# DanMcGann/loam

Measured on AMD Instinct MI355X. Metric: scan-pair registrations/sec (64x1024 Ouster), higher is better.
Workload: dtype f64; 1 GPU; batch of 1024 independent 64x1024 scan pairs per GPU (BASELINE configs[2]/[3]); step = extractFeatures x2 + registerFeatures per pair, inputs resident in HBM; pairs_per_gpu=1024, scan=64x1024, seed=20240311, input_scalar=f64, arithmetic=f64 (float input is widened on load)

## Files before the change

loam_amd/csrc/api_host.h:

```cpp
#pragma once
#include <math.h>
#include <stdio.h>
#include <stdlib.h>
#include <string.h>

#include <mutex>
#include <string>
#include <type_traits>
#include <utility>
#include <vector>

#include "loamx_internal.h"

namespace loamx {

enum WsId {
  WS_XYZ = 0, WS_CURV, WS_MASK,
  WS_SORT_SCRATCH, WS_SORT_SCRATCH_SRC, WS_NASSOC, WS_STATE, WS_PARTIALS, WS_MOM_PARTIALS, WS_MOMENTS, WS_FLAGGED_LIST, WS_FLAGGED_COUNT,
  WS_LINE_TOT, WS_EXTRACT_EVENTS, WS_BOX, WS_FINITE_FLAG, WS_COUNTERS, WS_ITERINFO, WS_STREAM_IN0, WS_STREAM_IN1, WS_STREAM_RES,
  WS_FIT_IN, WS_FIT_OUT, WS_FCOUNTS, WS_RESULTS, WS_INIT, WS_STREAM_INIT,
  WS_VOX_TABLE, WS_MAP_WORDS, WS_INFO_PARTIALS, WS_INFO,
  WS_COUNT
};
enum WsKindId {
  WSK_STAGE = 0, WSK_CNT, WSK_IDX, WSK_N, WSK_XYZ,
  WSK_GRID_DESC, WSK_CELLS, WSK_SORTED, WSK_REL, WSK_SGRID_DESC, WSK_SCELLS, WSK_SSORTED, WSK_ASSOC, WSK_NN, WSK_RNN, WSK_NEAREST,
  WSK_REST, WSK_EXACT, WSK_DUMP, WSK_SRC, WSK_TGT, WSK_MAP_TMP, WSK_MAP_OUT,
  WSK_COUNT
};

struct Buf {
  void* p = nullptr;
  size_t cap = 0;
};

struct PendingEvent {
  int kernel;
  hipEvent_t e0, e1;
  double bytes;
  bool own_e0;
};

}

struct loamx_ctx {
  int device = 0;
  hipStream_t own_stream = nullptr, stream = nullptr;
  bool max_counts_clean = false;
  hipStream_t aux_stream = nullptr;
  hipEvent_t ev_fork = nullptr, ev_mid = nullptr, ev_join = nullptr;
  hipEvent_t ev_counts = nullptr;
// ... 203 lines not shown
```

loam_amd/csrc/api_register.hip:

```cpp
#include "api_host.h"

using namespace loamx;

namespace {

int enqueue_association(loamx_ctx* ctx, const RegBatch& B, const RegConfig& C, uint32_t what = kAssocEdges | kAssocPlanes) {
  hipStream_t s = ctx->stream;
  {
    TimedScope t(ctx, LOAMX_K_ASSOC, 0.0);
    const bool side = (size_t)B.n_pairs * B.kind[kPlane].assoc_blocks >= 128;
    PendingEvent knn{};
    LaunchScope knn_ls{nullptr, nullptr, true};
    if (ctx->timing) {
      knn.kernel = LOAMX_K_KNN_PLANE, knn.bytes = 0.0, knn.own_e0 = true;
      knn.e0 = take_event(ctx), knn.e1 = take_event(ctx);
      knn_ls = LaunchScope{knn.e0, knn.e1, true};
    }
    launch_associate(B, C, s, side ? ctx->aux_stream : nullptr, side ? ctx->aux2_stream : nullptr, ctx->ev_fork, ctx->ev_mid, ctx->ev_join,
                     ctx->ev_join2, ctx->timing ? &knn_ls : nullptr, what);
    if (ctx->timing) {
      if (knn_ls.first) ctx->event_pool.push_back(knn.e0), ctx->event_pool.push_back(knn.e1);
      else ctx->pending.push_back(knn);
    }
  }
// ... 84 lines not shown
    ENSURE(ctx, b, bytes);
    if ((C.flags & kRegFlagPoison) && b.p) HIP_TRY(ctx, hipMemsetAsync(b.p, 0xFF, b.cap, ctx->stream));
    field = reinterpret_cast<std::remove_reference_t<decltype(field)>>(b.p);
    return LOAMX_OK;
  };
#define SCRATCH(buf, bytes, field)                \
  do {                                            \
    int rc_ = scratch(buf, bytes, field);         \
    if (rc_ != LOAMX_OK) return rc_;              \
  } while (0)
#define SCRATCH_K(id, bytes, field)                                                                        \
  for (int k = 0; k < 2; k++) {                                                                            \
    RegKind& K = B.kind[k];                                                                                \
    const size_t st = K.stride, km = C.kind[k].k <= 5 ? 5 : (C.kind[k].k <= 8 ? 8 : kMaxK), rec = k ? 7 : 9; \
    SCRATCH(ctx->wsk[id][k], bytes, K.field);                                                              \
  }
  SCRATCH_K(WSK_GRID_DESC, np * sizeof(GridDesc), grid.desc)
  SCRATCH_K(WSK_CELLS, (np * (size_t)(kGridCellsCap + 1) + 4) * sizeof(uint32_t), grid.cell_start)
  SCRATCH_K(WSK_SORTED, np * (st + kGridPad) * sizeof(GridPoint), grid.sorted)
  SCRATCH_K(WSK_REL, np * 3 * (st + kGridPad) * sizeof(float), grid.rel)
  SCRATCH_K(WSK_SGRID_DESC, np * sizeof(GridDesc), src_grid.desc)
  SCRATCH_K(WSK_SCELLS, np * (size_t)(kGridCellsCap + 1) * sizeof(uint32_t), src_grid.cell_start)
  SCRATCH_K(WSK_SSORTED, np * st * sizeof(GridPoint), src_grid.sorted)
  SCRATCH(ctx->ws[WS_SORT_SCRATCH], np * (es > ps ? es : ps) * sizeof(GridPoint), B.sort_scratch);
  SCRATCH(ctx->ws[WS_SORT_SCRATCH_SRC], grid_small(es > ps ? es : ps, C.flags) ? sizeof(GridPoint) : np * (es > ps ? es : ps) * sizeof(GridPoint), B.sort_scratch_src);
  SCRATCH_K(WSK_ASSOC, rec * np * st * sizeof(double), rec)
  SCRATCH_K(WSK_NN, (1 + km) * np * st * sizeof(uint32_t), nn)
  SCRATCH_K(WSK_RNN, (1 + km) * np * st * sizeof(uint32_t), rnn)
  SCRATCH_K(WSK_NEAREST, np * st * sizeof(uint32_t), nearest)
  SCRATCH_K(WSK_REST, np * st * sizeof(uint32_t), rest)
  SCRATCH_K(WSK_EXACT, np * st * sizeof(uint32_t), exact)
  SCRATCH(ctx->ws[WS_NASSOC], np * 8 * sizeof(uint32_t), B.n_assoc);
  SCRATCH(ctx->ws[WS_STATE], np * sizeof(PairState), B.state);
  SCRATCH(ctx->ws[WS_PARTIALS], np * B.blocks_per_pair * kAccSize * sizeof(double), B.partials);
  SCRATCH(ctx->ws[WS_MOM_PARTIALS], np * B.mom_blocks_per_pair * 4 * (size_t)(kMomSize + 2) * sizeof(double), B.mom_partials);
  SCRATCH(ctx->ws[WS_MOMENTS], np * (size_t)(kMomSize + 2) * sizeof(double), B.moments);
  SCRATCH(ctx->ws[WS_FLAGGED_LIST], np * (size_t)B.mom_blocks_per_pair * kSweepChunk * sizeof(uint32_t), B.flagged_list);
  SCRATCH(ctx->ws[WS_FLAGGED_COUNT], np * (size_t)B.mom_blocks_per_pair * 4 * sizeof(uint32_t), B.flagged_count);
  if (opts.want_info_partials) {
    InfoPartial* info_partials = nullptr;
    SCRATCH(ctx->ws[WS_INFO_PARTIALS], np * info_blocks_per_pair(es, ps) * sizeof(InfoPartial), info_partials);
  }
#undef SCRATCH_K
#undef SCRATCH
  {
    const bool fresh = ctx->ws[WS_COUNTERS].cap == 0;
    ENSURE(ctx, WS_COUNTERS, 128);
    untimed(ctx);
    if (fresh) HIP_TRY(ctx, hipMemsetAsync(ctx->ws[WS_COUNTERS].p, 0, 128, ctx->stream));
  }
  if (opts.want_iter_info) ENSURE(ctx, WS_ITERINFO, np * (size_t)(C.max_iterations ? C.max_iterations : 1) * sizeof(loamx_iter_info));
  B.n_active = wsp<uint32_t>(ctx, WS_COUNTERS);
  B.sweep_slots = reinterpret_cast<unsigned long long*>(wsp<unsigned char>(ctx, WS_COUNTERS) + 8);
  B.assoc_slots = B.sweep_slots + 2;
  B.grid_bytes = B.sweep_slots + 5;
  B.iter_info = opts.want_iter_info ? wsp<loamx_iter_info>(ctx, WS_ITERINFO) : nullptr;
  B.want_nearest = opts.want_nearest ? 1u : 0u;
  B.ref_moments = (C.flags & (kRegFlagNoMoments | kRegFlagNoRefMoments)) ? 0u : 1u;
  B.max_counts = wsp<uint32_t>(ctx, WS_COUNTERS) + 16;
  B.small_edge_sets = (C.flags & kRegFlagNoSmallSets) ? 0u : (!prebuilt ? 1u : (prebuilt->n[0] <= kBruteMax ? 2u : 0u));
  hipStream_t s = ctx->stream;
  untimed(ctx);
  if (!ctx->max_counts_clean) {
    const uint32_t init[6] = {0u, 0u, 0u, 0u, 0xFFFFFFFFu, 0xFFFFFFFFu};
    memcpy(&ctx->h_pinned[8], init, sizeof(init));
    HIP_TRY(ctx, hipMemcpyAsync(B.max_counts, &ctx->h_pinned[8], sizeof(init), hipMemcpyHostToDevice, s));
  }
  ctx->max_counts_clean = false;
  launch_state_init(B, C, s);
  CHECK_LAUNCH(ctx, "state_init_kernel");
  if (!ctx->ev_counts) HIP_TRY(ctx, hipEventCreateWithFlags(&ctx->ev_counts, hipEventDisableTiming));
  HIP_TRY(ctx, hipMemcpyAsync(&ctx->h_pinned[16], B.max_counts, 6 * sizeof(uint32_t), hipMemcpyDeviceToHost, s));
  HIP_TRY(ctx, hipEventRecord(ctx->ev_counts, s));

  if (prebuilt) {
    for (int k = 0; k < 2; k++) B.kind[k].grid = index_grid_set(prebuilt, k);
  }
  {
    TimedScope t(ctx, LOAMX_K_GRID, 0.0);
    const bool side = !(C.flags & kRegFlagNoGridSide) && ctx->aux_stream && !prebuilt && hipStreamWaitEvent(ctx->aux_stream, ctx->ev_counts, 0) == hipSuccess;
    if (!prebuilt) launch_grid_build_targets(B, C, s);
    launch_grid_build_sources(B, C, side ? ctx->aux_stream : s);
    if (side && hipEventRecord(ctx->ev_join, ctx->aux_stream) == hipSuccess) (void)hipStreamWaitEvent(s, ctx->ev_join, 0);
  }
  CHECK_LAUNCH(ctx, "grid_build_kernel");
// ... 435 lines not shown
```

loam_amd/csrc/info_kernels.hip:

```cpp
#include "loamx_internal.h"
#include "info_math.h"

namespace loamx {

namespace {

static_assert(sizeof(InfoPartial::s) == kInfoSums * sizeof(double), "InfoPartial holds the sums of info_math.h");
static_assert(sizeof(loamx_reg_information) == 696, "loamx.h documents the record's size");

constexpr int kInfoThreads = 256;
constexpr int kInfoItems = 16;
constexpr int kInfoChunk = kInfoThreads * kInfoItems;

__global__ void info_activate_kernel(RegBatch B) {
  const size_t pair = (size_t)blockIdx.x * blockDim.x + threadIdx.x;
  if (pair >= B.n_pairs) return;
  B.state[pair].active = 1u;
}

__global__ __launch_bounds__(kInfoThreads) void information_kernel(RegBatch B, InfoPartial* __restrict__ partials, uint32_t blocks_per_pair) {
  __shared__ double s_sum[kInfoThreads / 64][kInfoSums];
  __shared__ uint32_t s_cnt[kInfoThreads / 64][4];
  const size_t pair = blockIdx.x / blocks_per_pair;
  const uint32_t blk = blockIdx.x % blocks_per_pair;
  const uint32_t n_se_raw = B.kind[kEdge].n_src[pair * B.in_pitch], n_sp_raw = B.kind[kPlane].n_src[pair * B.in_pitch];
  const uint32_t n_se = n_se_raw < B.kind[kEdge].stride ? n_se_raw : (uint32_t)B.kind[kEdge].stride;
  const uint32_t n_sp = n_sp_raw < B.kind[kPlane].stride ? n_sp_raw : (uint32_t)B.kind[kPlane].stride;
  const uint32_t total = n_se + n_sp;
  const uint32_t base = blk * kInfoChunk;
  if (base >= total) return;
  const size_t efield = B.n_pairs * B.kind[kEdge].stride, pfield = B.n_pairs * B.kind[kPlane].stride;
  const double* __restrict__ E = B.kind[kEdge].rec + pair * B.kind[kEdge].stride;
  const double* __restrict__ Pl = B.kind[kPlane].rec + pair * B.kind[kPlane].stride;
  InfoAcc acc;
  info_acc_clear(acc);
  struct Rec {
    double f[9];
    int kind;
  };
  auto load_rec = [&](uint32_t v) {
    Rec R;
    R.kind = 0;
#pragma unroll
    for (int f = 0; f < 9; f++) R.f[f] = 0.0;
    if (v < total) {
      if (v < n_se) {
        R.kind = 1;
#pragma unroll
        for (int f = 0; f < 9; f++) R.f[f] = E[f * efield + v];
// ... 114 lines not shown
```

loam_amd/csrc/loamx_internal.h:

```cpp
#pragma once
#include <hip/hip_runtime.h>
#include <hip/hip_ext.h>
#include <stdint.h>
#include <stdio.h>

#include "../../include/loamx.h"
#include "extract_math.h"
#include "reg_math.h"

namespace loamx {

struct LaunchScope {
  hipEvent_t start, stop;
  bool first;
};
extern thread_local LaunchScope* g_launch_scope;
extern int g_debug_sync;
template <typename F, typename... Args>
inline void launch_kernel_named(const char* name, F kernel, const dim3& grid, const dim3& block, size_t shmem, hipStream_t s, Args... args) {
  LaunchScope* sc = g_launch_scope;
  if (g_debug_sync) fprintf(stderr, "[loamx] launch %s grid %u x %u block %u\n", name, grid.x, grid.y, block.x), fflush(stderr);
  if (sc) {
    hipExtLaunchKernelGGL(kernel, grid, block, (uint32_t)shmem, s, sc->first ? sc->start : nullptr, sc->stop, 0, args...);
    sc->first = false;
// ... 134 lines not shown
  uint32_t stream_planes;
  uint32_t use_moments;
  uint32_t mom_ref_on;
  double mom_ref[7];
};

constexpr int kSweepThreads = 256;
#ifndef LOAMX_SWEEP_ITEMS
#define LOAMX_SWEEP_ITEMS 16
#endif
constexpr int kSweepItems = LOAMX_SWEEP_ITEMS;
constexpr int kSweepChunk = kSweepThreads * kSweepItems;
constexpr uint32_t kEdgeCache = 320;
constexpr uint32_t kListCache = 64;
constexpr uint32_t kFlatCache = 192;

struct RegBatch {
  size_t n_pairs;
  uint32_t in_pitch;
  RegKind kind[2];
  const double* init;
  GridPoint* sort_scratch;
  GridPoint* sort_scratch_src;
  uint32_t* n_assoc;
  PairState* state;
  double* partials;
  double* mom_partials;
  double* moments;
  uint32_t mom_blocks_per_pair;
  uint32_t* flagged_list;
  uint32_t* flagged_count;
  uint32_t blocks_per_pair;
  uint32_t* n_active;
  unsigned long long* sweep_slots;
  unsigned long long* assoc_slots;
  unsigned long long* grid_bytes;
  loamx_iter_info* iter_info;
  uint32_t* max_counts;
  uint32_t want_nearest;
  uint32_t ref_moments;
  const unsigned long long* box_min;
  const unsigned long long* box_max;
  const uint32_t* box_bad;
  uint32_t src_box_offset;
  uint32_t small_edge_sets;
};

constexpr size_t kGridBigScratchBytes = 64 + ((size_t)kGridCellsCap + kGridCellsCap / 4096 + 8) * sizeof(uint32_t);
constexpr uint32_t kGridSmallCap = 20480;
constexpr uint32_t kBruteMax = 512;
constexpr uint32_t kGridMapCellsCap = 1u << 18;
inline bool grid_small(size_t stride, uint32_t reg_flags) { return stride <= kGridSmallCap && !(reg_flags & kRegFlagNoPackedGrid); }
void launch_grid_build_targets(const RegBatch& B, const RegConfig& C, hipStream_t s);
void launch_grid_build_sources(const RegBatch& B, const RegConfig& C, hipStream_t s);
constexpr uint32_t kGridBuildNone = 0u, kGridBuildPacked = 1u, kGridBuildSingle = 2u, kGridBuildBig = 3u;
struct GridBuildForm {
  uint32_t form;
  uint32_t unit_cells;
  uint32_t table_min_points;
};
GridBuildForm launch_grid_build_target(const RegBatch& B, const RegConfig& C, int kind, hipStream_t s);
void launch_grid_build_source(const RegBatch& B, const RegConfig& C, int kind, hipStream_t s);
void launch_state_init(const RegBatch& B, const RegConfig& C, hipStream_t s);
constexpr uint32_t kAssocEdges = 1u, kAssocPlanes = 2u;
void launch_associate(const RegBatch& B, const RegConfig& C, hipStream_t s, hipStream_t aux, hipStream_t aux2, hipEvent_t ev_fork,
                      hipEvent_t ev_mid, hipEvent_t ev_join, hipEvent_t ev_join2, LaunchScope* knn_scope = nullptr,
// ... 73 lines not shown
```

loam_amd/csrc/register_kernels.hip:

```cpp
#include "loamx_internal.h"

namespace loamx {

namespace {

__device__ __forceinline__ double wave_min(double v) {
#pragma unroll
  for (int off = 32; off >= 1; off >>= 1) v = fmin(v, __shfl_xor(v, off));
  return v;
}
__device__ __forceinline__ double wave_max(double v) {
#pragma unroll
  for (int off = 32; off >= 1; off >>= 1) v = fmax(v, __shfl_xor(v, off));
  return v;
}

#ifndef LOAMX_BUILD_THREADS
#define LOAMX_BUILD_THREADS 1024
#endif
constexpr int kBuildThreads = LOAMX_BUILD_THREADS;

template <bool ORDERED, bool PACKED>
__global__ __launch_bounds__(kBuildThreads) void grid_build_kernel(const double* __restrict__ pts_base,
                                                                   const uint32_t* __restrict__ n_pts, size_t stride,
// ... 549 lines not shown
  if (c <= ncell) cell_start[c] += shift[c];
  if (c < kGridPad) rel2[n_new + c] = kRelPad, rel2[stride + n_new + c] = kRelPad, rel2[2 * stride + n_new + c] = kRelPad;
  if (c == 0) desc->n_points = n_new;
}

constexpr int kRankThreads = 256;
__global__ __launch_bounds__(kRankThreads) void grid_rank_kernel(const uint32_t* __restrict__ n_pts, size_t stride,
                                                                 uint32_t in_pitch, GridSet gs,
                                                                 const GridPoint* __restrict__ scratch, const uint32_t* __restrict__ small_if) {
  const size_t pair = blockIdx.y;
  if (small_if && small_if[pair * in_pitch] <= kBruteMax) return;
  const uint32_t n_raw = n_pts[pair * in_pitch];
  const uint32_t n = n_raw < stride ? n_raw : (uint32_t)stride;
  const uint32_t p = blockIdx.x * kRankThreads + threadIdx.x;
  if (p >= n) return;
  const GridDesc g = gs.desc[pair];
  const uint32_t* __restrict__ cs = gs.cell_start + pair * (size_t)(kGridCellsCap + 1);
  const GridPoint* __restrict__ src = scratch + pair * gs.stride;
  GridPoint* __restrict__ sp = gs.sorted + pair * gs.stride;
  const GridPoint e = src[p];
  const uint32_t cell = grid_morton_of_point(g, v3(e.x, e.y, e.z));
  const uint32_t b = cs[cell], en = cs[cell + 1];
  uint32_t rank = 0;
#pragma unroll 4
  for (uint32_t j = b; j < en; j++) rank += src[j].orig < e.orig ? 1u : 0u;
  sp[b + rank] = e;
}

__global__ void state_init_kernel(RegBatch B, RegConfig C) {
  const size_t pair = (size_t)blockIdx.x * blockDim.x + threadIdx.x;
  if (pair >= B.n_pairs) return;
  PairState& S = B.state[pair];
  for (int i = 0; i < 7; i++) S.est[i] = B.init ? B.init[pair * 7 + i] : (i == 3 ? 1.0 : 0.0);
  S.active = C.max_iterations > 0 ? 1u : 0u;
  S.termination = LOAMX_MAX_ITER;
  S.iterations = 0;
  S.first_sweep = 0;
  S.stream_planes = 1;
  S.use_moments = 0;
  S.mom_ref_on = 0;
  S.lm.active = 0;
  for (int c = 0; c < 8; c++) B.n_assoc[8 * pair + c] = 0;
  if (B.max_counts) {
    const RegKind &E = B.kind[kEdge], &P = B.kind[kPlane];
    const uint32_t ne = E.n_src[pair * B.in_pitch], np = P.n_src[pair * B.in_pitch];
    atomicMax(&B.max_counts[0], ne < E.stride ? ne : (uint32_t)E.stride);
    atomicMax(&B.max_counts[1], np < P.stride ? np : (uint32_t)P.stride);
    if (E.n_tgt && P.n_tgt) {
      uint32_t te = E.n_tgt[pair * B.in_pitch], tp = P.n_tgt[pair * B.in_pitch];
      te = te < E.stride ? te : (uint32_t)E.stride, tp = tp < P.stride ? tp : (uint32_t)P.stride;
      atomicMax(&B.max_counts[2], te), atomicMax(&B.max_counts[3], tp);
      atomicMin(&B.max_counts[4], te), atomicMin(&B.max_counts[5], tp);
    }
  }
}

constexpr int kAssocThreads = 256;
#ifndef LOAMX_ASSOC_WAVES
#define LOAMX_ASSOC_WAVES 4
#endif
#ifndef LOAMX_KNN_REQUERY
#define LOAMX_KNN_REQUERY 1
#endif
#ifndef LOAMX_HANDOFF
#define LOAMX_HANDOFF 3
#endif
static_assert(!(LOAMX_HANDOFF & 2) || (LOAMX_HANDOFF & 1), "verification in the fit needs the threshold in front of the walk");
#ifndef LOAMX_ASSOC_WAVES5
#define LOAMX_ASSOC_WAVES5 (LOAMX_KNN_REQUERY ? 6 : 4)
#endif

__device__ __forceinline__ bool xcd_pair_map(uint32_t block, uint32_t blocks_per_pair, size_t n_pairs, size_t& pair,
                                             uint32_t& chunk) {
  if (n_pairs < 8) {
    pair = block / blocks_per_pair;
    chunk = block % blocks_per_pair;
  } else {
    const uint32_t xcd = block & 7u, slot = block >> 3;
    pair = (size_t)xcd + 8u * (size_t)(slot / blocks_per_pair);
    chunk = slot % blocks_per_pair;
  }
  return pair < n_pairs;
}

constexpr int kBruteTile = 256;
constexpr size_t kBruteLdsBytes = (kBruteTile + kGridPad) * sizeof(GridPoint) + ((3 * (kBruteTile + kGridPad) * sizeof(float) + 31) / 32) * 32;

template <class Coll>
__device__ __forceinline__ void brute_scan_tile(Coll& c, int k, Vec3 q, const GridPoint* s_tile, uint32_t tile, uint32_t tn) {
  for (uint32_t u = 0; u < tn; u += 4) {
    const GridPoint t0 = s_tile[u], t1 = s_tile[u + 1], t2 = s_tile[u + 2], t3 = s_tile[u + 3];
    double dx = q.x - t0.x, dy = q.y - t0.y, dz = q.z - t0.z;
    const double d0 = dx * dx + dy * dy + dz * dz;
    dx = q.x - t1.x, dy = q.y - t1.y, dz = q.z - t1.z;
    const double d1 = dx * dx + dy * dy + dz * dz;
    dx = q.x - t2.x, dy = q.y - t2.y, dz = q.z - t2.z;
    const double d2 = dx * dx + dy * dy + dz * dz;
    dx = q.x - t3.x, dy = q.y - t3.y, dz = q.z - t3.z;
    const double d3 = dx * dx + dy * dy + dz * dz;
    knn_offer4(c, k, d0, d1, d2, d3, tile + u, tn - u, t0.orig, t1.orig, t2.orig, t3.orig);
  }
}

template <bool PLANE, int KM>
__device__ __forceinline__ void knn_brute_body(const RegBatch& B, const RegConfig& C, uint32_t blocks_per_pair, uint32_t block,
                                               GridPoint* s_tile) {
  size_t pair;
  uint32_t chunk;
  if (!xcd_pair_map(block, blocks_per_pair, B.n_pairs, pair, chunk)) return;
  const PairState& S = B.state[pair];
  if (!S.active) return;
  const RegKind& K = B.kind[PLANE];
  const RegKindConfig& CK = C.kind[PLANE];
  const GridSet& gs = K.grid;
  const uint32_t n_tgt = gs.desc[pair].n_points;
  if (n_tgt > kBruteMax) return;
  const size_t stride = K.stride;
  const uint32_t n_src = K.n_src[pair * B.in_pitch];
  if (K.knn_mode == 2u && chunk == 0 && threadIdx.x == 0 && B.assoc_slots)
    atomicAdd(&B.assoc_slots[PLANE ? 1 : 0], (unsigned long long)(n_src < stride ? n_src : stride));
  if (chunk * kAssocThreads >= n_src || chunk * kAssocThreads >= stride) return;
  const uint32_t i = chunk * kAssocThreads + threadIdx.x;
  const bool has = i < n_src && i < stride;
  const GridSet& src_gs = K.src_grid;
  const GridPoint* __restrict__ sp = gs.sorted + pair * gs.stride;
  Vec3 p = v3(0, 0, 0);
  if (has) {
    const GridPoint sq = src_gs.sorted[pair * src_gs.stride + i];
    p = pose_act(S.est, v3(sq.x, sq.y, sq.z));
  }
  int k = CK.k;
  k = k < KM ? k : KM;
  const double max_dist = CK.r;
  uint32_t pos[KM];
#pragma unroll
  for (int j = 0; j < KM; j++) pos[j] = 0;
  int kept = 0;
  if (k > 0 && n_tgt > 0) {
    const double pass_max = CK.pass;
    kept = has ? -1 : 0;
    const GridDesc g = gs.desc[pair];
    if (gs.rel != nullptr && g.h > 0.0) {
// ... 74 lines not shown
      for (uint32_t tile = 0; tile < n_tgt; tile += kBruteTile) {
        const uint32_t tn = n_tgt - tile < (uint32_t)kBruteTile ? n_tgt - tile : (uint32_t)kBruteTile;
        __syncthreads();
        for (uint32_t t = threadIdx.x; t < tn + kGridPad; t += kAssocThreads) s_tile[t] = sp[tile + t];
        __syncthreads();
        if (kept < 0) brute_scan_tile(r, k, p, s_tile, tile, tn);
      }
      if (kept < 0) {
        kept = knn_finish(r, k, max_dist);
        knn_shift_positions<KM>(r.pos, k, pos);
      }
    }
  }
  if (!has) return;
  const size_t field = B.n_pairs * stride, slot = pair * stride + i;
  uint32_t* __restrict__ nn = K.nn;
  nn[slot] = (uint32_t)kept;
#pragma unroll
  for (int j = 0; j < KM; j++) nn[(1 + j) * field + slot] = pos[j];
}
template <bool PLANE, int KM>
__global__ __launch_bounds__(kAssocThreads) void associate_knn_brute_kernel(RegBatch B, RegConfig C, uint32_t blocks_per_pair) {
  __shared__ GridPoint s_tile[kBruteLdsBytes / sizeof(GridPoint)];
  knn_brute_body<PLANE, KM>(B, C, blocks_per_pair, blockIdx.x, s_tile);
}

constexpr uint32_t kQueueIndex = 0x3FFFFFFFu, kQueueWide = 0x80000000u, kQueueTied = 0x40000000u;

template <bool PLANE, int KM, int HANDOFF = 0>
__device__ __forceinline__ void knn_round1_body(const RegBatch& B, const RegConfig& C, uint32_t blocks_per_pair, uint32_t block,
                                                uint32_t* s_rows) {
  size_t pair;
  uint32_t chunk;
  if (!xcd_pair_map(block, blocks_per_pair, B.n_pairs, pair, chunk)) return;
  const uint32_t i = chunk * kAssocThreads + threadIdx.x;
  const PairState& S = B.state[pair];
  if (!S.active) return;
  const RegKind& K = B.kind[PLANE];
  const RegKindConfig& CK = C.kind[PLANE];
  const size_t stride = K.stride;
  const uint32_t n_src = K.n_src[pair * B.in_pitch];
  const GridSet &gs = K.grid, &src_gs = K.src_grid;
  if (chunk == 0 && threadIdx.x == 0 && B.assoc_slots)
    atomicAdd(&B.assoc_slots[PLANE ? 1 : 0], (unsigned long long)(n_src < stride ? n_src : stride));
  const GridDesc g = gs.desc[pair];
  if (g.n_points <= kBruteMax) return;
  if (i >= n_src || i >= stride) return;
  const GridPoint sq = src_gs.sorted[pair * src_gs.stride + i];
  const Vec3 p = pose_act(S.est, v3(sq.x, sq.y, sq.z));
  const uint32_t* __restrict__ cs = gs.cell_start + pair * (size_t)(kGridCellsCap + 1);
  const GridPoint* __restrict__ sp = gs.sorted + pair * gs.stride;
  uint32_t pos[KM];
  const float* __restrict__ rel = gs.rel + pair * 3 * gs.stride;
  const size_t field = B.n_pairs * stride;
  uint32_t word = 0;
#if LOAMX_KNN_REQUERY
  const GridPoint* __restrict__ src_pts = src_gs.sorted + pair * src_gs.stride;
  auto requery = [&](const Vec3&) -> Vec3 {
    uint32_t ii = i;
    asm volatile("" : "+v"(ii));
    const GridPoint s2 = src_pts[ii];
    return pose_act(S.est, v3(s2.x, s2.y, s2.z));
  };
  const int kept = knn_search_f32_round1<KM, false, decltype(requery), (HANDOFF & 3)>(g, cs, sp, rel, (uint32_t)gs.stride, p, CK.k,
                                             CK.r, CK.pass, pos, s_rows + threadIdx.x, kAssocThreads, requery, &word);
#else
  const int kept = knn_search_f32_round1<KM>(g, cs, sp, rel, (uint32_t)gs.stride, p, CK.k, CK.r, CK.pass, pos,
// ... 14 lines not shown
template <bool PLANE, int KM>
__global__ __launch_bounds__(kAssocThreads, KM <= 5 ? LOAMX_ASSOC_WAVES5 : LOAMX_ASSOC_WAVES) void associate_knn_kernel(RegBatch B, RegConfig C,
                                                                                         uint32_t blocks_per_pair) {
  __shared__ uint32_t s_rows[kLeanRowWords * kAssocThreads];
  knn_round1_body<PLANE, KM>(B, C, blocks_per_pair, blockIdx.x, s_rows);
}
template <int KME, int KMP>
__global__ __launch_bounds__(kAssocThreads, (KME <= 5 && KMP <= 5) ? LOAMX_ASSOC_WAVES5 : LOAMX_ASSOC_WAVES) void associate_knn_mixed_kernel(RegBatch B, RegConfig C, uint32_t blocks_edge,
                                                                                               uint32_t blocks_plane, uint32_t edge_blocks) {
  constexpr size_t kRowBytes = sizeof(uint32_t) * kLeanRowWords * kAssocThreads, kTileBytes = kBruteLdsBytes;
  __shared__ __attribute__((aligned(16))) unsigned char s_raw[kRowBytes > kTileBytes ? kRowBytes : kTileBytes];
  if (blockIdx.x < edge_blocks) knn_brute_body<false, KME>(B, C, blocks_edge, blockIdx.x, reinterpret_cast<GridPoint*>(s_raw));
  else knn_round1_body<true, KMP, LOAMX_HANDOFF>(B, C, blocks_plane, blockIdx.x - edge_blocks, reinterpret_cast<uint32_t*>(s_raw));
}

#ifndef LOAMX_REST_THREADS
#define LOAMX_REST_THREADS 64
#endif
constexpr int kRestThreads = LOAMX_REST_THREADS;
__host__ __device__ inline bool queue_leftovers_coop(const RegConfig& C, int kind) {
  return !(C.flags & kRegFlagNoCoopLeft) && C.kind[kind].r > 0.0;
}
#ifndef LOAMX_COOP_WAVES
#define LOAMX_COOP_WAVES 4
#endif
#define LOAMX_REST_WAVES(KM) ((KM) <= 8 ? 3 : 2)
constexpr int kLeftWaves = 5;
template <bool PLANE, int KM, bool ONE_STAGE>
__global__ __launch_bounds__(kRestThreads, LOAMX_REST_WAVES(KM)) void associate_knn_rest_kernel(RegBatch B, RegConfig C,
                                                                                              uint32_t blocks_per_pair) {
  constexpr bool one_stage = ONE_STAGE;
  size_t pair;
  uint32_t chunk0;
  if (!xcd_pair_map(blockIdx.x, blocks_per_pair, B.n_pairs, pair, chunk0)) return;
  const PairState& S = B.state[pair];
  if (!S.active) return;
  const uint32_t queued = B.n_assoc[8 * pair + (PLANE ? 3 : 2)];
  if (queued == 0u) return;
  __shared__ uint32_t s_rows[(ONE_STAGE ? kLeanRowWords : kLean2RowWords) * kRestThreads];
  const RegKind& K = B.kind[PLANE];
  const RegKindConfig& CK = C.kind[PLANE];
  const size_t stride = K.stride;
  const size_t field = B.n_pairs * stride;
  uint32_t* __restrict__ rnn = K.rnn;
  const uint32_t* __restrict__ rest = K.rest + pair * stride;
  uint32_t* __restrict__ left = K.exact + pair * stride;
  const GridSet &gs = K.grid, &src_gs = K.src_grid;
  const GridDesc g = gs.desc[pair];
  const uint32_t* __restrict__ cs = gs.cell_start + pair * (size_t)(kGridCellsCap + 1);
  const GridPoint* __restrict__ sp = gs.sorted + pair * gs.stride;
  const bool spread = B.n_pairs < 8 && (size_t)queued * 4 <= (size_t)blocks_per_pair * kRestThreads;
  const uint32_t t0 = spread ? chunk0 + blocks_per_pair * threadIdx.x : chunk0 * kRestThreads + threadIdx.x;
  const uint32_t dt = spread ? 0xFFFFFFFFu - t0 : blocks_per_pair * kRestThreads;
  const bool lean_set = g.n_points <= kLeanMaxPoints;
  const int kq = CK.k;
  const double max_dist = CK.r, pass_max = CK.pass;
  for (uint32_t t = t0; t < queued; t += dt) {
    const uint32_t entry = rest[t], i = entry & kQueueIndex;
    const size_t slot = pair * stride + t;
    uint32_t pos[KM];
#pragma unroll
    for (int j = 0; j < KM; j++) pos[j] = 0;
    int kept = -1;
    const bool coop = !one_stage && queue_leftovers_coop(C, PLANE);
    if (one_stage || (!(entry & kQueueTied) && ((lean_set && !(entry & kQueueWide)) || ((entry & kQueueWide) && !coop)))) {
      const GridPoint sq = src_gs.sorted[pair * src_gs.stride + i];
      const Vec3 p = pose_act(S.est, v3(sq.x, sq.y, sq.z));
      if (entry & kQueueWide)
        kept = knn_search_f32_round1<KM, true>(g, cs, sp, gs.rel + pair * 3 * gs.stride, (uint32_t)gs.stride, p, kq, max_dist, pass_max, pos,
                                                s_rows + threadIdx.x, kRestThreads);
      else if (!one_stage)
        kept = knn_lean_round2<KM>(g, cs, sp, gs.rel + pair * 3 * gs.stride, (uint32_t)gs.stride, p, kq, max_dist, pass_max, pos,
                                   s_rows + threadIdx.x, kRestThreads);
      if (one_stage && kept < 0)
        kept = knn_search_keyed<KM>(g, cs, sp, p, kq, max_dist, pass_max, pos, s_rows + threadIdx.x, kRestThreads);
    }
    rnn[slot] = (uint32_t)kept;
    if (kept < 0) left[atomicAdd(&B.n_assoc[8 * pair + (PLANE ? 5 : 4)], 1u)] = t;
#pragma unroll
    for (int j = 0; j < KM; j++) rnn[(1 + j) * field + slot] = pos[j];
  }
}

template <bool PLANE, int KM>
__global__ __launch_bounds__(kRestThreads, kLeftWaves) void associate_knn_left_kernel(RegBatch B, RegConfig C,
                                                                                              uint32_t blocks_per_pair) {
  size_t pair;
  uint32_t chunk0;
  if (!xcd_pair_map(blockIdx.x, blocks_per_pair, B.n_pairs, pair, chunk0)) return;
  const PairState& S = B.state[pair];
  if (!S.active) return;
  const uint32_t listed = B.n_assoc[8 * pair + (PLANE ? 5 : 4)];
  if (listed == 0u) return;
  __shared__ uint32_t s_rows[kLeanRowWords * kRestThreads];
  const RegKind& K = B.kind[PLANE];
  const RegKindConfig& CK = C.kind[PLANE];
  const size_t stride = K.stride;
  const size_t field = B.n_pairs * stride;
  uint32_t* __restrict__ rnn = K.rnn;
  const uint32_t* __restrict__ rest = K.rest + pair * stride;
  const uint32_t* __restrict__ left = K.exact + pair * stride;
  const GridSet &gs = K.grid, &src_gs = K.src_grid;
  const GridDesc g = gs.desc[pair];
  const uint32_t* __restrict__ cs = gs.cell_start + pair * (size_t)(kGridCellsCap + 1);
  const GridPoint* __restrict__ sp = gs.sorted + pair * gs.stride;
  const bool spread = B.n_pairs < 8 && (size_t)listed * 4 <= (size_t)blocks_per_pair * kRestThreads;
  const uint32_t t0 = spread ? chunk0 + blocks_per_pair * threadIdx.x : chunk0 * kRestThreads + threadIdx.x;
  const uint32_t dt = spread ? 0xFFFFFFFFu - t0 : blocks_per_pair * kRestThreads;
  for (uint32_t t = t0; t < listed; t += dt) {
    const uint32_t qpos = left[t], i = rest[qpos] & kQueueIndex;
    const size_t slot = pair * stride + qpos;
    const GridPoint sq = src_gs.sorted[pair * src_gs.stride + i];
    const Vec3 p = pose_act(S.est, v3(sq.x, sq.y, sq.z));
    uint32_t pos[KM];
    const int kept = knn_search_keyed<KM>(g, cs, sp, p, CK.k, CK.r, CK.pass, pos, s_rows + threadIdx.x, kRestThreads);
    rnn[slot] = (uint32_t)kept;
#pragma unroll
    for (int j = 0; j < KM; j++) rnn[(1 + j) * field + slot] = pos[j];
  }
}

constexpr int32_t kCoopMaxShell = 64;
// ... 141 lines not shown
        bound = ub < bound ? ub : bound;
      }
      done = knn_done(g, q, k, max_dist, cx, cy, cz, probe, w);
    }
  }
  if (!done) return -1;
  KnnKeys<KM> m;
  knn_init(m, k, g.n_points);
#pragma unroll
  for (int t = 0; t <= KM; t++) {
    if (t >= KM - k) {
      double head = knn_key_empty();
#pragma unroll
      for (int j = KM; j >= 0; j--)
        if (j >= KM - k) head = c.key[j] < head ? c.key[j] : head;
      const double best = wave_min_all(head);
      m.key[t] = best;
      if (head == best && best < knn_key_empty()) {
#pragma unroll
        for (int j = 0; j < KM; j++)
          if (j >= KM - k) c.key[j] = c.key[j + 1];
        c.key[KM] = knn_key_empty();
      }
    }
  }
  return knn_keys_finish(m, k, pass_max, pos);
}

static_assert(kRestThreads == 64, "associate_knn_coop_kernel is written for one wavefront per workgroup");
template <bool PLANE, int KM>
__global__ __launch_bounds__(kRestThreads, LOAMX_COOP_WAVES) void associate_knn_coop_kernel(RegBatch B, RegConfig C, uint32_t blocks_per_pair) {
  size_t pair;
  uint32_t chunk0;
  if (!xcd_pair_map(blockIdx.x, blocks_per_pair, B.n_pairs, pair, chunk0)) return;
  const PairState& S = B.state[pair];
  if (!S.active) return;
  const uint32_t listed = B.n_assoc[8 * pair + (PLANE ? 5 : 4)];
  if (listed == 0u) return;
  __shared__ uint32_t s_rows[kLeanRowWords];
  const RegKind& K = B.kind[PLANE];
  const RegKindConfig& CK = C.kind[PLANE];
  const size_t stride = K.stride;
  const size_t field = B.n_pairs * stride;
  uint32_t* __restrict__ rnn = K.rnn;
  const uint32_t* __restrict__ rest = K.rest + pair * stride;
  const uint32_t* __restrict__ left = K.exact + pair * stride;
  const GridSet &gs = K.grid, &src_gs = K.src_grid;
  const GridDesc g = gs.desc[pair];
  const uint32_t* __restrict__ cs = gs.cell_start + pair * (size_t)(kGridCellsCap + 1);
  const GridPoint* __restrict__ sp = gs.sorted + pair * gs.stride;
  const int kq = CK.k;
  const double max_dist = CK.r, pass_max = CK.pass;
  for (uint32_t t = chunk0; t < listed; t += blocks_per_pair) {
    const uint32_t qpos = left[t], i = rest[qpos] & kQueueIndex;
    const size_t slot = pair * stride + qpos;
    const GridPoint sq = src_gs.sorted[pair * src_gs.stride + i];
    const Vec3 p = pose_act(S.est, v3(sq.x, sq.y, sq.z));
    uint32_t pos[KM];
    int kept = knn_coop_search<KM>(g, cs, sp, p, kq, max_dist, pass_max, pos);
    if (kept == -2) {
      if ((threadIdx.x & 63) == 0) kept = knn_search_keyed<KM>(g, cs, sp, p, kq, max_dist, pass_max, pos, s_rows, 1);
      kept = __builtin_amdgcn_readfirstlane(kept);
#pragma unroll
      for (int j = 0; j < KM; j++) pos[j] = (uint32_t)__builtin_amdgcn_readfirstlane((int)pos[j]);
    }
    if ((threadIdx.x & 63) == 0) {
      rnn[slot] = (uint32_t)kept;
// ... 65 lines not shown
#pragma unroll
    for (int j = 0; j < KM; j++) nb[j] = j < kept ? v3(tp[j].x, tp[j].y, tp[j].z) : v3(0, 0, 0);
    if (kept > 0) nearest = tp[0].orig;
    if (PLANE) {
      Vec3 nrm;
      double d;
      const double avg = fit_plane<KM>(nb, kept, nrm, d);
      valid = !(avg > C.max_avg_plane_dist);
      prim[0] = nrm.x, prim[1] = nrm.y, prim[2] = nrm.z, prim[3] = d;
    } else {
      Vec3 a, b;
      fit_line<KM>(nb, kept, a, b);
      valid = !(kDblMax < C.min_line_cond);
      prim[0] = a.x, prim[1] = a.y, prim[2] = a.z, prim[3] = b.x, prim[4] = b.y, prim[5] = b.z;
    }
  }
  double* __restrict__ rec = K.rec;
  rec[slot] = valid ? p.x : __longlong_as_double(0x7FF8000000000000ll);
  rec[field + slot] = p.y;
  rec[2 * field + slot] = p.z;
#pragma unroll
  for (int f = 0; f < (PLANE ? 4 : 6); f++) rec[(3 + f) * field + slot] = prim[f];
  if (B.want_nearest) K.nearest[pair * stride + sq.orig] = valid ? nearest : 0xFFFFFFFFu;
  return valid;
}

#ifndef LOAMX_FIT_WAVES
#define LOAMX_FIT_WAVES 4
#endif
template <bool PLANE, int KM, int HANDOFF = 0>
__device__ __forceinline__ void fit_body(const RegBatch& B, const RegConfig& C, uint32_t blocks_per_pair, uint32_t block) {
  size_t pair;
  uint32_t chunk;
  if (!xcd_pair_map(block, blocks_per_pair, B.n_pairs, pair, chunk)) return;
  const uint32_t i = chunk * kAssocThreads + threadIdx.x;
  const PairState& S = B.state[pair];
  if (!S.active) return;
  const RegKind& K = B.kind[PLANE];
  const size_t stride = K.stride;
  const uint32_t n_src = K.n_src[pair * B.in_pitch];
  const uint32_t* nn = K.nn;
  bool valid = false;
  if (i < n_src && i < stride) valid = fit_one<PLANE, KM, false, HANDOFF>(B, C, S, pair, i, nn, pair * stride + i);
  const unsigned long long m = __ballot(valid);
  if ((threadIdx.x & 63) == 0 && m) atomicAdd(&B.n_assoc[8 * pair + (PLANE ? 1 : 0)], (uint32_t)__popcll(m));
}
template <bool PLANE, int KM>
__global__ __launch_bounds__(kAssocThreads, LOAMX_FIT_WAVES) void associate_fit_kernel(RegBatch B, RegConfig C,
                                                                                        uint32_t blocks_per_pair) {
  fit_body<PLANE, KM>(B, C, blocks_per_pair, blockIdx.x);
}
template <int KME, int KMP>
__global__ __launch_bounds__(kAssocThreads, LOAMX_FIT_WAVES) void associate_fit_mixed_kernel(RegBatch B, RegConfig C, uint32_t blocks_edge,
                                                                                              uint32_t blocks_plane, uint32_t edge_blocks) {
  if (blockIdx.x < edge_blocks) fit_body<false, KME>(B, C, blocks_edge, blockIdx.x);
  else fit_body<true, KMP, LOAMX_HANDOFF>(B, C, blocks_plane, blockIdx.x - edge_blocks);
}

template <bool PLANE, int KM>
__global__ __launch_bounds__(kRestThreads, 3) void associate_fit_queued_kernel(RegBatch B, RegConfig C, uint32_t blocks_per_pair) {
  size_t pair;
  uint32_t chunk0;
  if (!xcd_pair_map(blockIdx.x, blocks_per_pair, B.n_pairs, pair, chunk0)) return;
  const PairState& S = B.state[pair];
  if (!S.active) return;
  const uint32_t queued = B.n_assoc[8 * pair + (PLANE ? 3 : 2)];
  if (queued == 0u) return;
  __shared__ uint32_t s_rows[18 * kRestThreads];
  const RegKind& K = B.kind[PLANE];
  const size_t stride = K.stride;
  uint32_t* rnn = K.rnn;
  const uint32_t* __restrict__ rest = K.rest + pair * stride;
  uint32_t count = 0;
  for (uint32_t t = chunk0 * kRestThreads + threadIdx.x; t < queued; t += blocks_per_pair * kRestThreads) {
    const uint32_t i = rest[t] & kQueueIndex;
    if ((int)rnn[pair * stride + t] < 0)
      knn_exact_one<PLANE, KM>(B, C, S, pair, i, pair * stride + t, rnn, s_rows + threadIdx.x, kRestThreads);
    count += fit_one<PLANE, KM, true>(B, C, S, pair, i, rnn, pair * stride + t) ? 1u : 0u;
  }
#pragma unroll
  for (int off = 32; off >= 1; off >>= 1) count += __shfl_xor(count, off);
  if ((threadIdx.x & 63) == 0 && count) atomicAdd(&B.n_assoc[8 * pair + (PLANE ? 1 : 0)], count);
}

template <bool PLANE, int KM>
__global__ __launch_bounds__(kRestThreads, 3) void associate_fit_late_kernel(RegBatch B, RegConfig C, uint32_t blocks_per_pair) {
  size_t pair;
  uint32_t chunk0;
  if (!xcd_pair_map(blockIdx.x, blocks_per_pair, B.n_pairs, pair, chunk0)) return;
  const uint32_t late = B.n_assoc[8 * pair + 6 + (PLANE ? 1 : 0)];
  if (late == 0u) return;
  const PairState& S = B.state[pair];
  if (!S.active) return;
  __shared__ uint32_t s_rows[18 * kRestThreads];
  const RegKind& K = B.kind[PLANE];
  const size_t stride = K.stride;
  uint32_t* nn = K.nn;
  const uint32_t* __restrict__ list = K.exact + pair * stride;
  uint32_t count = 0;
  for (uint32_t t = chunk0 * kRestThreads + threadIdx.x; t < late && t < stride; t += blocks_per_pair * kRestThreads) {
    const uint32_t i = list[stride - 1 - t];
    knn_exact_one<PLANE, KM>(B, C, S, pair, i, pair * stride + i, nn, s_rows + threadIdx.x, kRestThreads);
    count += fit_one<PLANE, KM, true>(B, C, S, pair, i, nn, pair * stride + i) ? 1u : 0u;
  }
#pragma unroll
  for (int off = 32; off >= 1; off >>= 1) count += __shfl_xor(count, off);
  if ((threadIdx.x & 63) == 0 && count) atomicAdd(&B.n_assoc[8 * pair + (PLANE ? 1 : 0)], count);
}

__global__ __launch_bounds__(64) void lm_begin_kernel(RegBatch B, RegConfig C) {
  const size_t pair = (size_t)blockIdx.x * blockDim.x + threadIdx.x;
  if (pair >= B.n_pairs) return;
  if (pair == 0) *B.n_active = 0u;
  PairState& S = B.state[pair];
  if (!S.active) return;
  const uint32_t iteration = S.iterations;
  const uint32_t ne = B.n_assoc[8 * pair], np = B.n_assoc[8 * pair + 1];
  for (int c = 0; c < 8; c++) B.n_assoc[8 * pair + c] = 0;
  if ((uint64_t)ne + np < C.min_associations) {
    S.termination = LOAMX_INSUFFICIENT_ASSOCIATIONS;
    S.active = 0;
    S.lm.active = 0;
// ... 265 lines not shown
  S.lm = lm;
  S.first_sweep = 0;
  if (first && B.ref_moments && !S.use_moments && lm.active) {
    S.use_moments = 1u, S.mom_ref_on = 1u;
    for (int i = 0; i < 7; i++) S.mom_ref[i] = lm.xeval[i];
    S.stream_planes = 1u;
    return;
  }
  const bool valid = S.mom_ref_on ? plane_moments_valid_rel(mom[kMomSize], mom[kMomSize + 1], lm.xeval, S.mom_ref)
                                  : plane_moments_valid_at(mom[kMomSize], mom[kMomSize + 1], lm.xeval);
  S.stream_planes = (!S.use_moments || (lm.active && !valid)) ? 1u : 0u;
}

__global__ __launch_bounds__(64) void lm_step_kernel(RegBatch B) {
  const size_t pair = (size_t)blockIdx.x * blockDim.x + threadIdx.x;
  if (pair >= B.n_pairs) return;
  PairState& S = B.state[pair];
  if (!S.active || !S.lm.active) return;
  const uint32_t n_se_raw = B.kind[kEdge].n_src[pair * B.in_pitch], n_sp_raw = B.kind[kPlane].n_src[pair * B.in_pitch];
  const uint32_t n_se = n_se_raw < B.kind[kEdge].stride ? n_se_raw : (uint32_t)B.kind[kEdge].stride;
  const uint32_t n_sp = n_sp_raw < B.kind[kPlane].stride ? n_sp_raw : (uint32_t)B.kind[kPlane].stride;
  const uint32_t used = S.stream_planes ? (n_se + n_sp + kSweepChunk - 1) / kSweepChunk : 1u;
  double acc[kAccSize];
  for (int j = 0; j < kAccSize; j++) acc[j] = 0.0;
  for (uint32_t b = 0; b < used && b < B.blocks_per_pair; b++) {
    const double* __restrict__ p = B.partials + (pair * B.blocks_per_pair + b) * kAccSize;
    for (int j = 0; j < kAccSize; j++) acc[j] += p[j];
  }
  lm_step_pair(B, pair, S, acc);
}

__device__ __forceinline__ void outer_update_pair(const RegBatch& B, const RegConfig& C, size_t pair, PairState& S) {
  const uint32_t iteration = S.iterations;
  double upd[7];
  for (int i = 0; i < 7; i++) upd[i] = S.lm.x_user[i];
  if (B.iter_info) {
    loamx_iter_info& I = B.iter_info[pair * C.max_iterations + iteration];
    for (int i = 0; i < 7; i++) I.estimate_update[i] = upd[i];
  }
  S.iterations = iteration + 1;
  double est[7];
  for (int i = 0; i < 7; i++) est[i] = S.est[i];
  const bool converged = outer_update(est, upd, C.rot_thresh, C.pos_thresh);
  S.use_moments = (C.flags & kRegFlagNoMoments) ? 0u : 1u;
  for (int i = 0; i < 7; i++) S.est[i] = est[i];
  if (converged) {
    S.termination = LOAMX_CONVERGED;
    S.active = 0;
  } else if (iteration + 1 >= C.max_iterations) {
    S.active = 0;
  } else {
    atomicAdd(B.n_active, 1u);
  }
}

__global__ __launch_bounds__(64) void lm_pair_loop_kernel(RegBatch B, RegConfig C) {
  __shared__ LightLds L;
  __shared__ double s_mom[kMomSize + 2];
  __shared__ double s_acc[kAccSize];
  __shared__ double s_edge[9][kEdgeCache];
  __shared__ double s_frec[7][kFlatCache];
  __shared__ uint32_t s_listed[kListCache], s_pref[kListCache];
  const int lane = threadIdx.x;
  const size_t pair = blockIdx.x;
  PairState& S_global = B.state[pair];
  if (!S_global.active) return;
  if (!S_global.lm.active) {
    if (lane == 0) outer_update_pair(B, C, pair, S_global);
    return;
  }
  __shared__ PairState s_S;
  static_assert(sizeof(PairState) % 8 == 0, "copied as 64-bit words");
  {
    const unsigned long long* __restrict__ src = reinterpret_cast<const unsigned long long*>(&S_global);
    unsigned long long* dst = reinterpret_cast<unsigned long long*>(&s_S);
    for (int w = lane; w < (int)(sizeof(PairState) / 8); w += 64) dst[w] = src[w];
  }
  wave_lds_fence();
  PairState& S = s_S;
  const uint32_t n_se_raw = B.kind[kEdge].n_src[pair * B.in_pitch], n_sp_raw = B.kind[kPlane].n_src[pair * B.in_pitch];
  const uint32_t n_se = n_se_raw < B.kind[kEdge].stride ? n_se_raw : (uint32_t)B.kind[kEdge].stride;
  const uint32_t n_sp = n_sp_raw < B.kind[kPlane].stride ? n_sp_raw : (uint32_t)B.kind[kPlane].stride;
  {
    const size_t efield = B.n_pairs * B.kind[kEdge].stride;
    const double* __restrict__ E = B.kind[kEdge].rec + pair * B.kind[kEdge].stride;
// ... 669 lines not shown
```

Baseline: 105,200 pairs/s.

## Compact still-active pairs into a live list and remap association blocks onto it

The outer update now appends each still-iterating pair to a device-side live list through the active-count atomic and sets a validity flag. The block-to-pair mapping in the association, KNN and fit kernels then maps block slots onto only the listed live pairs and exits the rest early. This avoids spreading blocks over pairs that have already converged in later iterations. It adds two global loads per block, and correctness depends on the list and the counter staying consistent with the launch grid. Work assigned to dead pairs is skipped rather than redistributed.

```diff
diff --git a/loam_amd/csrc/api_host.h b/loam_amd/csrc/api_host.h
--- a/loam_amd/csrc/api_host.h
+++ b/loam_amd/csrc/api_host.h
@@ -16,7 +16,7 @@
 
 enum WsId {
   WS_XYZ = 0, WS_CURV, WS_MASK,
-  WS_SORT_SCRATCH, WS_SORT_SCRATCH_SRC, WS_NASSOC, WS_STATE, WS_PARTIALS, WS_MOM_PARTIALS, WS_MOMENTS, WS_FLAGGED_LIST, WS_FLAGGED_COUNT,
+  WS_SORT_SCRATCH, WS_SORT_SCRATCH_SRC, WS_NASSOC, WS_STATE, WS_LIVE_LIST, WS_PARTIALS, WS_MOM_PARTIALS, WS_MOMENTS, WS_FLAGGED_LIST, WS_FLAGGED_COUNT,
   WS_LINE_TOT, WS_EXTRACT_EVENTS, WS_BOX, WS_FINITE_FLAG, WS_COUNTERS, WS_ITERINFO, WS_STREAM_IN0, WS_STREAM_IN1, WS_STREAM_RES,
   WS_FIT_IN, WS_FIT_OUT, WS_FCOUNTS, WS_RESULTS, WS_INIT, WS_STREAM_INIT,
   WS_VOX_TABLE, WS_MAP_WORDS, WS_INFO_PARTIALS, WS_INFO,
diff --git a/loam_amd/csrc/api_register.hip b/loam_amd/csrc/api_register.hip
--- a/loam_amd/csrc/api_register.hip
+++ b/loam_amd/csrc/api_register.hip
@@ -140,6 +140,7 @@
   SCRATCH_K(WSK_EXACT, np * st * sizeof(uint32_t), exact)
   SCRATCH(ctx->ws[WS_NASSOC], np * 8 * sizeof(uint32_t), B.n_assoc);
   SCRATCH(ctx->ws[WS_STATE], np * sizeof(PairState), B.state);
+  SCRATCH(ctx->ws[WS_LIVE_LIST], np * sizeof(uint32_t), B.live_list);
   SCRATCH(ctx->ws[WS_PARTIALS], np * B.blocks_per_pair * kAccSize * sizeof(double), B.partials);
   SCRATCH(ctx->ws[WS_MOM_PARTIALS], np * B.mom_blocks_per_pair * 4 * (size_t)(kMomSize + 2) * sizeof(double), B.mom_partials);
   SCRATCH(ctx->ws[WS_MOMENTS], np * (size_t)(kMomSize + 2) * sizeof(double), B.moments);
@@ -159,6 +160,7 @@
   }
   if (opts.want_iter_info) ENSURE(ctx, WS_ITERINFO, np * (size_t)(C.max_iterations ? C.max_iterations : 1) * sizeof(loamx_iter_info));
   B.n_active = wsp<uint32_t>(ctx, WS_COUNTERS);
+  B.live_valid = B.n_active + 1;
   B.sweep_slots = reinterpret_cast<unsigned long long*>(wsp<unsigned char>(ctx, WS_COUNTERS) + 8);
   B.assoc_slots = B.sweep_slots + 2;
   B.grid_bytes = B.sweep_slots + 5;
diff --git a/loam_amd/csrc/info_kernels.hip b/loam_amd/csrc/info_kernels.hip
--- a/loam_amd/csrc/info_kernels.hip
+++ b/loam_amd/csrc/info_kernels.hip
@@ -15,6 +15,7 @@
 __global__ void info_activate_kernel(RegBatch B) {
   const size_t pair = (size_t)blockIdx.x * blockDim.x + threadIdx.x;
   if (pair >= B.n_pairs) return;
+  if (pair == 0) *B.live_valid = 0u;
   B.state[pair].active = 1u;
 }
 
diff --git a/loam_amd/csrc/loamx_internal.h b/loam_amd/csrc/loamx_internal.h
--- a/loam_amd/csrc/loamx_internal.h
+++ b/loam_amd/csrc/loamx_internal.h
@@ -190,6 +190,8 @@
   uint32_t* flagged_count;
   uint32_t blocks_per_pair;
   uint32_t* n_active;
+  uint32_t* live_list;
+  uint32_t* live_valid;
   unsigned long long* sweep_slots;
   unsigned long long* assoc_slots;
   unsigned long long* grid_bytes;
diff --git a/loam_amd/csrc/register_kernels.hip b/loam_amd/csrc/register_kernels.hip
--- a/loam_amd/csrc/register_kernels.hip
+++ b/loam_amd/csrc/register_kernels.hip
@@ -605,6 +605,7 @@
   if (pair >= B.n_pairs) return;
   PairState& S = B.state[pair];
   for (int i = 0; i < 7; i++) S.est[i] = B.init ? B.init[pair * 7 + i] : (i == 3 ? 1.0 : 0.0);
+  if (pair == 0) *B.live_valid = 0u;
   S.active = C.max_iterations > 0 ? 1u : 0u;
   S.termination = LOAMX_MAX_ITER;
   S.iterations = 0;
@@ -643,8 +644,8 @@
 #define LOAMX_ASSOC_WAVES5 (LOAMX_KNN_REQUERY ? 6 : 4)
 #endif
 
-__device__ __forceinline__ bool xcd_pair_map(uint32_t block, uint32_t blocks_per_pair, size_t n_pairs, size_t& pair,
-                                             uint32_t& chunk) {
+__device__ __forceinline__ bool xcd_pair_map(const RegBatch& B, uint32_t block, uint32_t blocks_per_pair, size_t& pair, uint32_t& chunk) {
+  const size_t n_pairs = B.n_pairs;
   if (n_pairs < 8) {
     pair = block / blocks_per_pair;
     chunk = block % blocks_per_pair;
@@ -652,6 +653,12 @@
     const uint32_t xcd = block & 7u, slot = block >> 3;
     pair = (size_t)xcd + 8u * (size_t)(slot / blocks_per_pair);
     chunk = slot % blocks_per_pair;
+    const uint32_t listed = B.live_list[pair < n_pairs ? pair : n_pairs - 1];
+    const uint32_t valid = *B.live_valid, n_live = *B.n_active;
+    if (valid) {
+      if (pair >= n_live) return false;
+      pair = listed;
+    }
   }
   return pair < n_pairs;
 }
@@ -680,7 +687,7 @@
                                                GridPoint* s_tile) {
   size_t pair;
   uint32_t chunk;
-  if (!xcd_pair_map(block, blocks_per_pair, B.n_pairs, pair, chunk)) return;
+  if (!xcd_pair_map(B, block, blocks_per_pair, pair, chunk)) return;
   const PairState& S = B.state[pair];
   if (!S.active) return;
   const RegKind& K = B.kind[PLANE];
@@ -821,7 +828,7 @@
                                                 uint32_t* s_rows) {
   size_t pair;
   uint32_t chunk;
-  if (!xcd_pair_map(block, blocks_per_pair, B.n_pairs, pair, chunk)) return;
+  if (!xcd_pair_map(B, block, blocks_per_pair, pair, chunk)) return;
   const uint32_t i = chunk * kAssocThreads + threadIdx.x;
   const PairState& S = B.state[pair];
   if (!S.active) return;
@@ -902,7 +909,7 @@
   constexpr bool one_stage = ONE_STAGE;
   size_t pair;
   uint32_t chunk0;
-  if (!xcd_pair_map(blockIdx.x, blocks_per_pair, B.n_pairs, pair, chunk0)) return;
+  if (!xcd_pair_map(B, blockIdx.x, blocks_per_pair, pair, chunk0)) return;
   const PairState& S = B.state[pair];
   if (!S.active) return;
   const uint32_t queued = B.n_assoc[8 * pair + (PLANE ? 3 : 2)];
@@ -957,7 +964,7 @@
                                                                                               uint32_t blocks_per_pair) {
   size_t pair;
   uint32_t chunk0;
-  if (!xcd_pair_map(blockIdx.x, blocks_per_pair, B.n_pairs, pair, chunk0)) return;
+  if (!xcd_pair_map(B, blockIdx.x, blocks_per_pair, pair, chunk0)) return;
   const PairState& S = B.state[pair];
   if (!S.active) return;
   const uint32_t listed = B.n_assoc[8 * pair + (PLANE ? 5 : 4)];
@@ -1165,7 +1172,7 @@
 __global__ __launch_bounds__(kRestThreads, LOAMX_COOP_WAVES) void associate_knn_coop_kernel(RegBatch B, RegConfig C, uint32_t blocks_per_pair) {
   size_t pair;
   uint32_t chunk0;
-  if (!xcd_pair_map(blockIdx.x, blocks_per_pair, B.n_pairs, pair, chunk0)) return;
+  if (!xcd_pair_map(B, blockIdx.x, blocks_per_pair, pair, chunk0)) return;
   const PairState& S = B.state[pair];
   if (!S.active) return;
   const uint32_t listed = B.n_assoc[8 * pair + (PLANE ? 5 : 4)];
@@ -1297,7 +1304,7 @@
 __device__ __forceinline__ void fit_body(const RegBatch& B, const RegConfig& C, uint32_t blocks_per_pair, uint32_t block) {
   size_t pair;
   uint32_t chunk;
-  if (!xcd_pair_map(block, blocks_per_pair, B.n_pairs, pair, chunk)) return;
+  if (!xcd_pair_map(B, block, blocks_per_pair, pair, chunk)) return;
   const uint32_t i = chunk * kAssocThreads + threadIdx.x;
   const PairState& S = B.state[pair];
   if (!S.active) return;
@@ -1326,7 +1333,7 @@
 __global__ __launch_bounds__(kRestThreads, 3) void associate_fit_queued_kernel(RegBatch B, RegConfig C, uint32_t blocks_per_pair) {
   size_t pair;
   uint32_t chunk0;
-  if (!xcd_pair_map(blockIdx.x, blocks_per_pair, B.n_pairs, pair, chunk0)) return;
+  if (!xcd_pair_map(B, blockIdx.x, blocks_per_pair, pair, chunk0)) return;
   const PairState& S = B.state[pair];
   if (!S.active) return;
   const uint32_t queued = B.n_assoc[8 * pair + (PLANE ? 3 : 2)];
@@ -1352,7 +1359,7 @@
 __global__ __launch_bounds__(kRestThreads, 3) void associate_fit_late_kernel(RegBatch B, RegConfig C, uint32_t blocks_per_pair) {
   size_t pair;
   uint32_t chunk0;
-  if (!xcd_pair_map(blockIdx.x, blocks_per_pair, B.n_pairs, pair, chunk0)) return;
+  if (!xcd_pair_map(B, blockIdx.x, blocks_per_pair, pair, chunk0)) return;
   const uint32_t late = B.n_assoc[8 * pair + 6 + (PLANE ? 1 : 0)];
   if (late == 0u) return;
   const PairState& S = B.state[pair];
@@ -1684,6 +1691,7 @@
 
 __device__ __forceinline__ void outer_update_pair(const RegBatch& B, const RegConfig& C, size_t pair, PairState& S) {
   const uint32_t iteration = S.iterations;
+  *B.live_valid = 1u;
   double upd[7];
   for (int i = 0; i < 7; i++) upd[i] = S.lm.x_user[i];
   if (B.iter_info) {
@@ -1702,7 +1710,8 @@
   } else if (iteration + 1 >= C.max_iterations) {
     S.active = 0;
   } else {
-    atomicAdd(B.n_active, 1u);
+    const uint32_t at = atomicAdd(B.n_active, 1u);
+    if (at < B.n_pairs) B.live_list[at] = (uint32_t)pair;
   }
 }
 
```

New measurement: 105,200 pairs/s, median of 2. No clear change (-0.0%).
